# interactiveaudiolab/ppgs

Hardware: AMD Instinct MI355X
Metric: PPG frames/sec (whole node), mel repr, batch=32x1000 frames (higher is better)
Workload: dtype bf16; 1 GPU; configs[1]: mel representation, batch=32 x 1000 frames per GPU, audio resident in HBM -> (32,40,1000) fp32 posteriors in HBM; batch=32, frames=1000, per_gpu_batches=1, parallelism=utterance-sharded x1, no data-path collective

## Files before the change

### ppgs_amd/csrc/ppg_layer32.h

```cpp
#pragma once

#include "ppg_device.h"
#include "ppg_launch.h"

#include <type_traits>
#include <utility>

namespace {

constexpr float kLnEps32 = 1e-5f;
constexpr int HC = 128;

constexpr int tile_blocks(int hidt) { return hidt == 256 ? 5 : 3; }
template <int HIDT, int TBN_ = tile_blocks(HIDT)>
struct Geo {
    static_assert(HIDT == 256 || HIDT == 512, "hidden width");
    static constexpr int RB = HIDT / 128;
    static constexpr int KS = HIDT / 16;
    static constexpr int KH = KS / 16;
    static constexpr int TBN = TBN_;
    static constexpr int TOKS = 32 * TBN;
    static constexpr int HBUFS = TBN_ == tile_blocks(HIDT) ? 1 : 2;
    static constexpr int L_ACT = 0;
    static constexpr int L_H = TBN * KS * 1024;
    static constexpr int L_LNP1 = L_H + HBUFS * TBN * 8 * 1024;
    static constexpr int L_LNP2 = L_LNP1 + 3 * HIDT * 4;
    static constexpr int L_BQ = L_LNP2 + 3 * HIDT * 4;
    static constexpr int L_STATS = L_BQ + 3 * HIDT * 4;
    static constexpr int L_B1 = L_STATS + 2 * 4 * TOKS * 4;
};

__device__ __forceinline__ uint32_t lds_addr32(const void* p) {
    return (uint32_t)(uintptr_t)(const __attribute__((address_space(3))) void*)p;
}
template <int OFF>
__device__ __forceinline__ void ds_read128(u32x4& dst, uint32_t addr) {
    asm volatile("ds_read_b128 %0, %1 offset:%2" : "=v"(dst) : "v"(addr), "n"(OFF));
}
template <int N>
__device__ __forceinline__ void lgkm_wait32(u32x4& r) {
    asm volatile("s_waitcnt lgkmcnt(%1)" : "+v"(r) : "n"(N) : "memory");
    __builtin_amdgcn_sched_barrier(0);
}
template <int OFF>
__device__ __forceinline__ void gload128(u32x4& dst, uint32_t voff, const char* sbase) {
    asm volatile("global_load_dwordx4 %0, %1, %2 offset:%3" : "=v"(dst) : "v"(voff), "s"(sbase), "n"(OFF) : "memory");
}
template <int OFF>
__device__ __forceinline__ void gload128_acc(u32x4& dst, uint32_t voff, const char* sbase) {
    asm volatile("global_load_dwordx4 %0, %1, %2 offset:%3" : "=a"(dst) : "v"(voff), "s"(sbase), "n"(OFF) : "memory");
}
template <int K>
__device__ __forceinline__ void gload_frag(u32x4& dst, uint32_t voff, const char* base) {
    gload128<(K % 4) * 1024>(dst, voff, base + (K / 4) * 4096);
}
template <int K>
__device__ __forceinline__ void gload_frag_acc(u32x4& dst, uint32_t voff, const char* base) {
    gload128_acc<(K % 4) * 1024>(dst, voff, base + (K / 4) * 4096);
}
template <int COUNT>
__device__ __forceinline__ void vm_wait_all(u32x4 (&r)[COUNT]) {
    asm volatile("s_waitcnt vmcnt(0)" ::: "memory");
#pragma unroll
    for (int i = 0; i < COUNT; ++i) asm volatile("" : "+v"(r[i]));
    __builtin_amdgcn_sched_barrier(0);
}
__device__ __forceinline__ void glds16(const char* uniform_base, uint32_t lane_off, uint32_t lds_wave_addr) {
    const uint64_t b = reinterpret_cast<uint64_t>(uniform_base);
    const uint64_t base = ((uint64_t)(uint32_t)__builtin_amdgcn_readfirstlane((int)(b >> 32)) << 32) |
                          (uint64_t)(uint32_t)__builtin_amdgcn_readfirstlane((int)(uint32_t)b);
    asm volatile("s_mov_b32 m0, %2\n\ts_nop 0\n\tglobal_load_lds_dwordx4 %0, %1"
                 :: "v"(lane_off), "s"(base), "s"(__builtin_amdgcn_readfirstlane(lds_wave_addr)) : "memory", "m0");
}

template <class OFFS, int I, int N, int D, class USE>
__device__ __forceinline__ void stream_step(u32x4 (&ring)[D], uint32_t b0, uint32_t b1, USE& use) {
    if constexpr (I < N) {
        lgkm_wait32<(N - 1 - I < D - 1) ? (N - 1 - I) : (D - 1)>(ring[I % D]);
        use(std::integral_constant<int, I>{}, ring[I % D]);
        if constexpr (I + D < N) {
            constexpr int off = OFFS::at(I + D);
            if constexpr (off < 65536) ds_read128<off>(ring[I % D], b0); else ds_read128<off - 65536>(ring[I % D], b1);
        }
        stream_step<OFFS, I + 1, N, D>(ring, b0, b1, use);
    }
}
template <class OFFS, int I, int N, int D>
__device__ __forceinline__ void stream_prime(u32x4 (&ring)[D], uint32_t b0, uint32_t b1) {
    if constexpr (I < D && I < N) {
        constexpr int off = OFFS::at(I);
        if constexpr (off < 65536) ds_read128<off>(ring[I], b0); else ds_read128<off - 65536>(ring[I], b1);
        stream_prime<OFFS, I + 1, N, D>(ring, b0, b1);
    }
}
template <class OFFS, int N, int D, class USE>
__device__ __forceinline__ void stream(uint32_t b0, uint32_t b1, USE use) {
    u32x4 ring[D];
    stream_prime<OFFS, 0, N, D>(ring, b0, b1);
    stream_step<OFFS, 0, N, D>(ring, b0, b1, use);
}
template <int KS, int K0, int TB0, int NTB>
struct OffPanel { static constexpr int at(int i) { return ((TB0 + i % NTB) * KS + K0 + i / NTB) * 1024; } };
template <int TBN>
struct OffH { static constexpr int at(int i) { return ((i % TBN) * 8 + i / TBN) * 1024; } };

template <int TBN, int PAR>
struct OffH2 { static constexpr int at(int i) { return PAR * (TBN * 8 * 1024) + ((i % TBN) * 8 + i / TBN) * 1024; } };

struct OffChunk256 {
    static constexpr int at(int i) {
        constexpr int KS = Geo<256>::KS, HOFF = Geo<256>::L_H - Geo<256>::L_ACT;
        if (i < 48) return ((i % 3) * KS + i / 3) * 1024;
        if (i < 80) return ((3 + (i - 48) % 2) * KS + (i - 48) / 2) * 1024;
        if (i < 104) return HOFF + (((i - 80) % 3) * 8 + (i - 80) / 3) * 1024;
        return HOFF + ((3 + (i - 104) % 2) * 8 + (i - 104) / 2) * 1024;
    }
};

__device__ __forceinline__ void stat4(f32x2& sum2, f32x2& sq2, float v0, float v1, float v2, float v3) {
    const f32x2 a = {v0, v1}, b = {v2, v3};
    sum2 += a;
    sq2 = __builtin_elementwise_fma(a, a, sq2);
    sum2 += b;
    sq2 = __builtin_elementwise_fma(b, b, sq2);
}
__device__ __forceinline__ float hsum2(f32x2 v) {
    float r;
    asm("v_add_f32 %0, %1, %2" : "=v"(r) : "v"(v.x), "v"(v.y));
    return r;
}
__device__ __forceinline__ float pair_sum(float v) {
    auto b = __builtin_amdgcn_permlane32_swap(__float_as_uint(v), __float_as_uint(v), false, false);
    return __uint_as_float(b[0]) + __uint_as_float(b[1]);
}

template <class P, int HIDT, int TBS = tile_blocks(HIDT)>
__device__ __forceinline__ void panel_store(uint32_t pb0, int wave, int t, int rb, const f32x16& y) {
    using G = Geo<HIDT, TBS>;
#pragma unroll
    for (int s = 0; s < 2; ++s) {
        const u32x4 frag = u32x4{P::pack2(y[8 * s + 0], y[8 * s + 1]), P::pack2(y[8 * s + 2], y[8 * s + 3]),
                                 P::pack2(y[8 * s + 4], y[8 * s + 5]), P::pack2(y[8 * s + 6], y[8 * s + 7])};
        const uint32_t addr = pb0 + (uint32_t)((t * G::KS + 2 * G::RB * wave + 2 * rb + s) * 1024);
        asm volatile("ds_write_b128 %0, %1" :: "v"(addr), "v"(frag) : "memory");
    }
}

template <class P, int HIDT, int TBS = tile_blocks(HIDT)>
__device__ __forceinline__ void qkv_tail(const Layer32Args& a, char* smem, const int m0, u32x4 (&w1f)[16], u32x4 (&w2f)[16],
                                         const int nblk = TBS) {
    using G = Geo<HIDT, TBS>;
    constexpr int RB = G::RB, KS = G::KS, KH = G::KH, TB = G::TBN, TOKS = G::TOKS;
    constexpr int NSTEP = 3 * RB, NHS = NSTEP * KH;
    constexpr int NMMA = 16 * TB;
    constexpr int NU = 2 * TB;
    constexpr int USTRIDE = (NMMA - 16) / NU;
    const int lane = threadIdx.x & 63;
    const int wave = __builtin_amdgcn_readfirstlane(threadIdx.x >> 6);
    const int tok = lane & 31, hh = lane >> 5;
    const uint32_t voff = lane * 16;
    const uint32_t pb0 = lds_addr32(smem) + G::L_ACT + lane * 16, pb1 = pb0 + 65536;
    const int fbase = 32 * RB * wave;
    const f32x16 zero = {0.f, 0.f, 0.f, 0.f, 0.f, 0.f, 0.f, 0.f, 0.f, 0.f, 0.f, 0.f, 0.f, 0.f, 0.f, 0.f};
    asm volatile("s_waitcnt lgkmcnt(0)" ::: "memory");
    __syncthreads();
    const float* bq = reinterpret_cast<const float*>(smem + G::L_BQ);
    int vcol[TB][2];
    bool valigned[TB];
    bool regular = m0 + TOKS <= a.M && nblk == TB;
#pragma unroll
    for (int t = 0; t < TB; ++t) {
#pragma unroll
        for (int h = 0; h < 2; ++h) {
            const int mb = m0 + 32 * t + 16 * h;
            vcol[t][h] = -1;
            if (mb < a.M && t < nblk) {
                const int w = a.blk_win[mb >> 4];
                if (w >= 0) {
                    const int ttb = mb - a.win[w].tok_off;
                    vcol[t][h] = a.win[w].vt_off + (ttb >> 5) * 32 + 4 * ((ttb >> 4) & 1);
                }
            }
        }
        valigned[t] = vcol[t][0] >= 0 && vcol[t][1] == vcol[t][0] + 4 && (vcol[t][0] & 31) == 0;
        regular = regular && valigned[t];
    }
    const char* wq = a.wq_img + ((size_t)wave * 3 * RB * KS) * 1024;
    f32x16 acc[2][TB];
    auto bias_of = [&](auto step_tag, float4 (&b4)[4]) {
        constexpr int STEP = decltype(step_tag)::value, KIND = STEP / RB, RBI = STEP % RB;
        if constexpr (KIND < 2) {
#pragma unroll
            for (int q = 0; q < 4; ++q) b4[q] = *reinterpret_cast<const float4*>(bq + HIDT * KIND + 32 * RBI + fbase + 16 * hh + 4 * q);
        } else {
            const float bv = bq[2 * HIDT + pair_row(fbase + 32 * RBI + tok)];
            b4[0] = make_float4(bv, bv, bv, bv);
        }
    };
    auto bias_c = [&](auto step_tag) {
        constexpr int STEP = decltype(step_tag)::value;
        f32x16 cinit = zero;
        float4 bb[4];
        bias_of(step_tag, bb);
        if constexpr (STEP / RB < 2) {
#pragma unroll
            for (int q = 0; q < 4; ++q) { cinit[4 * q + 0] = bb[q].x; cinit[4 * q + 1] = bb[q].y; cinit[4 * q + 2] = bb[q].z; cinit[4 * q + 3] = bb[q].w; }
        } else {
#pragma unroll
            for (int k = 0; k < 16; ++k) cinit[k] = bb[0].x;
        }
        return cinit;
    };
    u32x4 held = u32x4{0u, 0u, 0u, 0u};
    auto unit = [&](auto step_tag, auto u_tag) {
        constexpr int STEP = decltype(step_tag)::value, U = decltype(u_tag)::value;
        constexpr int KIND = STEP / RB, RBI = STEP % RB, t = U / 2, s2 = U % 2;
        const f32x16& c = acc[STEP & 1][t];
        if (regular) {
            u32x4 r;
            if constexpr (KIND < 2) {
                r = u32x4{P::pack2(c[8 * s2 + 0], c[8 * s2 + 1]),
                          P::pack2(c[8 * s2 + 2], c[8 * s2 + 3]),
                          P::pack2(c[8 * s2 + 4], c[8 * s2 + 5]),
                          P::pack2(c[8 * s2 + 6], c[8 * s2 + 7])};
            } else {
                r = u32x4{P::pack2(c[4 * s2 + 0], c[4 * s2 + 1]), P::pack2(c[4 * s2 + 2], c[4 * s2 + 3]),
                          P::pack2(c[4 * (s2 + 2) + 0], c[4 * (s2 + 2) + 1]), P::pack2(c[4 * (s2 + 2) + 2], c[4 * (s2 + 2) + 3])};
            }
            if constexpr (s2 == 0) {
                held = r;
            } else {
                u32x4 lo, hi;
#pragma unroll
                for (int d = 0; d < 4; ++d) {
                    const auto sw = __builtin_amdgcn_permlane16_swap(held[d], r[d], false, false);
                    lo[d] = sw[0]; hi[d] = sw[1];
                }
                const int r16 = lane & 15, k16 = lane >> 4;
                if constexpr (KIND < 2) {
                    char* dst = a.qk_out + ((size_t)(m0 + 32 * t + r16) * 2 * HIDT + HIDT * KIND + 32 * RBI + fbase) * 2 + 16 * k16;
                    *reinterpret_cast<u32x4*>(dst) = lo;
                    *reinterpret_cast<u32x4*>(dst + (size_t)16 * 2 * HIDT * 2) = hi;
                } else {
                    char* dst = a.vt_out + ((size_t)(fbase + 32 * RBI + r16) * a.vt_ld + vcol[t][0]) * 2 + 16 * (2 * (k16 & 1) + (k16 >> 1));
                    *reinterpret_cast<u32x4*>(dst) = lo;
                    *reinterpret_cast<u32x4*>(dst + (size_t)16 * a.vt_ld * 2) = hi;
                }
            }
            return;
        }
        if constexpr (KIND < 2) {
            const int m = m0 + 32 * t + tok;
            if (m < a.M && t < nblk) {
                char* dst = a.qk_out + ((size_t)m * 2 * HIDT + HIDT * KIND + 32 * RBI + fbase + 16 * hh) * 2;
                *reinterpret_cast<u32x4*>(dst + 16 * s2) = u32x4{
                    P::pack2(c[8 * s2 + 0], c[8 * s2 + 1]), P::pack2(c[8 * s2 + 2], c[8 * s2 + 3]),
                    P::pack2(c[8 * s2 + 4], c[8 * s2 + 5]), P::pack2(c[8 * s2 + 6], c[8 * s2 + 7])};
            }
        } else {
            char* rowp = a.vt_out + (size_t)(fbase + 32 * RBI + tok) * a.vt_ld * 2;
            if (valigned[t]) {
                *reinterpret_cast<u32x4*>(rowp + (size_t)(vcol[t][0] + 16 * s2 + 8 * hh) * 2) = u32x4{
                    P::pack2(c[4 * s2 + 0], c[4 * s2 + 1]), P::pack2(c[4 * s2 + 2], c[4 * s2 + 3]),
                    P::pack2(c[4 * (s2 + 2) + 0], c[4 * (s2 + 2) + 1]), P::pack2(c[4 * (s2 + 2) + 2], c[4 * (s2 + 2) + 3])};
            } else if (vcol[t][s2] >= 0) {
#pragma unroll
                for (int e = 0; e < 2; ++e) {
                    const int q = 2 * s2 + e;
                    *reinterpret_cast<uint2*>(rowp + (size_t)(vcol[t][s2] + 8 * (2 * e + hh)) * 2) = make_uint2(
                        P::pack2(c[4 * q + 0], c[4 * q + 1]), P::pack2(c[4 * q + 2], c[4 * q + 3]));
                }
            }
        }
    };
    auto half_step = [&](auto hs_tag, u32x4 (&cur)[16], u32x4 (&nxt)[16]) {
        constexpr int HS = decltype(hs_tag)::value;
        constexpr int STEP = HS / KH, kh = HS % KH;
        constexpr bool SWAP = STEP / RB == 2;
        constexpr bool LAST = HS + 1 == NHS;
        constexpr bool EPI = kh == 0 && STEP > 0;
        const char* nbase = wq + (size_t)(LAST ? HS : HS + 1) * 16 * 1024;
        f32x16 cinit = zero;
        if constexpr (kh == 0) {
            cinit = bias_c(std::integral_constant<int, STEP>{});
#pragma unroll
            for (int k = 0; k < 16; ++k) asm volatile("" : "+v"(cinit[k]));
        }
        f32x16 (&c)[TB] = acc[STEP & 1];
        stream<OffPanel<KS, 16 * kh, 0, TB>, NMMA, 6>(pb0, pb1, [&](auto ic, const u32x4& bf) {
            constexpr int i = decltype(ic)::value;
            constexpr int ks = i / TB, tb = i % TB;
            if constexpr (ks == 0 && kh == 0) c[tb] = SWAP ? P::mma32(bf, cur[0], cinit) : P::mma32(cur[0], bf, cinit);
            else c[tb] = SWAP ? P::mma32(bf, cur[ks], c[tb]) : P::mma32(cur[ks], bf, c[tb]);
            if constexpr (!LAST && i < 16) gload_frag<i>(nxt[i], voff, nbase);
            if constexpr (EPI && i >= 16 && (i - 16) % USTRIDE == 0 && (i - 16) / USTRIDE < NU)
                unit(std::integral_constant<int, STEP - 1>{}, std::integral_constant<int, (i - 16) / USTRIDE>{});
        });
        if constexpr (!LAST) {
            if constexpr (EPI) {
                if (regular) asm volatile("s_waitcnt vmcnt(%0)" :: "n"(NU) : "memory");
                else asm volatile("s_waitcnt vmcnt(0)" ::: "memory");
            } else {
                asm volatile("s_waitcnt vmcnt(0)" ::: "memory");
            }
#pragma unroll
            for (int k = 0; k < 16; ++k) asm volatile("" : "+v"(nxt[k]));
            __builtin_amdgcn_sched_barrier(0);
        }
    };
    [&]<int... S>(std::integer_sequence<int, S...>) {
        ((S % 2 == 0 ? half_step(std::integral_constant<int, S>{}, w1f, w2f)
                     : half_step(std::integral_constant<int, S>{}, w2f, w1f)), ...);
    }(std::make_integer_sequence<int, NHS>{});
    (void)TOKS;
    [&]<int... U>(std::integer_sequence<int, U...>) {
        (unit(std::integral_constant<int, NSTEP - 1>{}, std::integral_constant<int, U>{}), ...);
    }(std::make_integer_sequence<int, NU>{});
}

}
```

### ppgs_amd/csrc/ppg_layer32.hip

```cpp
#include "ppg_layer32.h"

namespace {

template <class P, int HIDT, bool QKV, int TBS = tile_blocks(HIDT)>
__global__ __launch_bounds__(256) __attribute__((amdgpu_waves_per_eu(1, 1))) void layer32_kernel(Layer32Args a) {
    using G = Geo<HIDT, TBS>;
    constexpr int RB = G::RB, KS = G::KS, KH = G::KH, TB = G::TBN, TOKS = G::TOKS;
    constexpr int TBT = tile_blocks(HIDT);
    constexpr bool SUB = TBS != TBT;
    constexpr int NSUB = (TBT + TBS - 1) / TBS;
    static_assert(!SUB || (HIDT == 256 && TBS == 2), "sub-tile workgroups: hidden 256, two token blocks");
    extern __shared__ __attribute__((aligned(16))) char smem[];
    const int tid = threadIdx.x;
    const int lane = tid & 63;
    const int wave = __builtin_amdgcn_readfirstlane(tid >> 6);
    const int tok = lane & 31, hh = lane >> 5;
    const int tile = SUB ? (int)blockIdx.x / NSUB : (int)blockIdx.x;
    const int tb0 = SUB ? ((int)blockIdx.x % NSUB) * TBS : 0;
    const int nblk = SUB ? min(TBS, TBT - tb0) : TBS;
    auto gblock = [&](int t) { return SUB ? tb0 + (t < nblk ? t : -tb0) : t; };
    const int m0 = tile * (32 * TBT) + 32 * tb0;
    const int NCH = a.F / HC;
    const uint32_t lds0 = lds_addr32(smem);
    const uint32_t voff = lane * 16;
    const uint32_t pb0 = lds0 + G::L_ACT + lane * 16, pb1 = pb0 + 65536;
    const uint32_t hb0 = lds0 + G::L_H + lane * 16;
    float* lnp1 = reinterpret_cast<float*>(smem + G::L_LNP1);
    float* lnp2 = reinterpret_cast<float*>(smem + G::L_LNP2);
    float* stats = reinterpret_cast<float*>(smem + G::L_STATS);
    const int fbase = 32 * RB * wave;
    [[maybe_unused]] const char* wq_first = a.wq_img + ((size_t)wave * 3 * RB * KS) * 1024;

#ifdef PPG_FFN_TIMING
    auto pstamp = [&](int k) {
        if (a.dbg && blockIdx.x == 0 && lane == 0) a.dbg[128 + wave * 16 + k] = __builtin_amdgcn_s_memtime();
    };
#else
    auto pstamp = [&](int) {};
#endif
    pstamp(0);

    u32x4 w1f[16], w2f[16];
    auto load16 = [&](u32x4 (&wf)[16], const char* base) {
        [&]<int... K>(std::integer_sequence<int, K...>) { (gload_frag<K>(wf[K], voff, base), ...); }(std::make_integer_sequence<int, 16>{});
    };
    constexpr bool XPRE = HIDT == 256;
    constexpr int NRES = XPRE ? TB * RB * 2 : 1;
    u32x4 res[NRES];
    const bool xpre = XPRE && a.x_half;
    if (xpre) {
        const char* xbase = reinterpret_cast<const char*>(a.X) + ((size_t)tile * 4 + wave) * (TBT * RB * 2 * 1024);
        if constexpr (!SUB) {
            [&]<int... K>(std::integer_sequence<int, K...>) { (gload_frag<K>(res[K], voff, xbase), ...); }(std::make_integer_sequence<int, NRES>{});
        } else {
            [&]<int... K>(std::integer_sequence<int, K...>) {
                (gload_frag<K % (RB * 2)>(res[K], voff, xbase + (size_t)gblock(K / (RB * 2)) * (RB * 2 * 1024)), ...);
            }(std::make_integer_sequence<int, NRES>{});
        }
    }
    {
        const char* src = a.ao + (size_t)tile * (TBT * KS * 1024);
#pragma unroll
        for (int i = 0; i < TB * KS / 4; ++i) {
            const int p = 4 * i + wave;
            const int q = SUB ? gblock(p / KS) * KS + p % KS : p;
            glds16(src + (size_t)q * 1024, voff, lds0 + G::L_ACT + p * 1024);
        }
    }
    f32x16 yacc[RB][TB];
    {
        constexpr int NP = (3 * HIDT / 4 + 255) / 256;
        float4 p1[NP], p2[NP], pq[NP];
#pragma unroll
        for (int u = 0; u < NP; ++u) {
            const int i = min(tid + 256 * u, 3 * HIDT / 4 - 1);
            const int v = i / (HIDT / 4), j = i - v * (HIDT / 4);
            p1[u] = reinterpret_cast<const float4*>(v == 0 ? a.bo : (v == 1 ? a.g1 : a.e1))[j];
            p2[u] = reinterpret_cast<const float4*>(v == 0 ? a.b2 : (v == 1 ? a.g2 : a.e2))[j];
            if constexpr (QKV) pq[u] = reinterpret_cast<const float4*>(a.bq)[i];
        }
        constexpr int B1MAX = 8;
        float4 pb[B1MAX];
#pragma unroll
        for (int u = 0; u < B1MAX; ++u) pb[u] = reinterpret_cast<const float4*>(a.b1)[min(tid + 256 * u, a.F / 4 - 1)];
#pragma unroll
        for (int u = 0; u < NP; ++u) {
            const int i = tid + 256 * u;
            if (i < 3 * HIDT / 4) {
                reinterpret_cast<float4*>(lnp1)[i] = p1[u];
                reinterpret_cast<float4*>(lnp2)[i] = p2[u];
                if constexpr (QKV) reinterpret_cast<float4*>(smem + G::L_BQ)[i] = pq[u];
            }
        }
#pragma unroll
        for (int u = 0; u < B1MAX; ++u)
            if (tid + 256 * u < a.F / 4) reinterpret_cast<float4*>(smem + G::L_B1)[tid + 256 * u] = pb[u];
    }
    const f32x16 zero = {0.f, 0.f, 0.f, 0.f, 0.f, 0.f, 0.f, 0.f, 0.f, 0.f, 0.f, 0.f, 0.f, 0.f, 0.f, 0.f};
    [&]<int... R>(std::integer_sequence<int, R...>) {
        ([&] {
            constexpr int rbp = R / KH, kh = R % KH;
            const char* base = a.wo_img + ((size_t)wave * RB * KS) * 1024;
            load16(w1f, base + ((size_t)(2 * rbp) * KS + 16 * kh) * 1024);
            load16(w2f, base + ((size_t)(2 * rbp + 1) * KS + 16 * kh) * 1024);
            vm_wait_all(w1f);
            vm_wait_all(w2f);
            if constexpr (R == 0) {
#pragma unroll
                for (int k = 0; k < NRES; ++k) asm volatile("" : "+v"(res[k]));
                __syncthreads();
                pstamp(1);
            }
            if (!(PPG_DBG(a) & 1)) {
                stream<OffPanel<KS, 16 * kh, 0, TB>, 16 * TB, 6>(pb0, pb1, [&](auto ic, const u32x4& bf) {
                    constexpr int i = decltype(ic)::value;
                    constexpr int ks = i / TB, tb = i % TB;
                    if constexpr (ks == 0 && kh == 0) {
                        yacc[2 * rbp][tb] = P::mma32(w1f[0], bf, zero);
                        yacc[2 * rbp + 1][tb] = P::mma32(w2f[0], bf, zero);
                    } else {
                        yacc[2 * rbp][tb] = P::mma32(w1f[ks], bf, yacc[2 * rbp][tb]);
                        yacc[2 * rbp + 1][tb] = P::mma32(w2f[ks], bf, yacc[2 * rbp + 1][tb]);
                    }
                });
            }
        }(), ...);
    }(std::make_integer_sequence<int, (RB / 2) * KH>{});
    pstamp(2);

    float* xt = a.X + ((size_t)tile * 4 + wave) * (TBT * RB * 4 * 256) + lane * 4;
    char* xh = reinterpret_cast<char*>(a.X) + ((size_t)tile * 4 + wave) * (TBT * RB * 2 * 1024) + lane * 16;
    auto layer_norm = [&](auto residual_tag, auto xhalf_tag, const float* lnp, auto emit) {
        constexpr bool RES = decltype(residual_tag)::value;
        constexpr bool XH = decltype(xhalf_tag)::value;
        constexpr int STAMP = RES ? 7 : 9;
        constexpr bool KEEP = RB == 2;
        float4 bias4[KEEP ? RB : 1][4], gv[KEEP ? RB : 1][4], ev[KEEP ? RB : 1][4];
        auto quad = [&](int which, int rb, int q) { return *reinterpret_cast<const float4*>(lnp + which * HIDT + fbase + 32 * rb + 16 * hh + 4 * q); };
        if constexpr (KEEP) {
#pragma unroll
            for (int rb = 0; rb < RB; ++rb)
#pragma unroll
                for (int q = 0; q < 4; ++q) bias4[rb][q] = quad(0, rb, q);
        }
#pragma unroll
        for (int t = 0; t < TB; ++t) {
            f32x2 sum2 = {0.f, 0.f}, sq2 = {0.f, 0.f};
#pragma unroll
            for (int rb = 0; rb < RB; ++rb)
#pragma unroll
                for (int s2 = 0; s2 < 2; ++s2) {
                    float r8[8] = {0.f, 0.f, 0.f, 0.f, 0.f, 0.f, 0.f, 0.f};
                    [[maybe_unused]] uint32_t w4[4] = {0u, 0u, 0u, 0u};
                    if constexpr (RES && XH) {
                        u32x4 rv;
                        if constexpr (XPRE) rv = res[(t * RB + rb) * 2 + s2];
                        else rv = *reinterpret_cast<const u32x4*>(xh + ((gblock(t) * RB + rb) * 2 + s2) * 1024);
                        w4[0] = rv.x; w4[1] = rv.y; w4[2] = rv.z; w4[3] = rv.w;
                    } else if constexpr (RES) {
#pragma unroll
                        for (int e = 0; e < 2; ++e) {
                            const float4 rv = *reinterpret_cast<const float4*>(xt + ((gblock(t) * RB + rb) * 4 + 2 * s2 + e) * 256);
                            r8[4 * e + 0] = rv.x; r8[4 * e + 1] = rv.y; r8[4 * e + 2] = rv.z; r8[4 * e + 3] = rv.w;
                        }
                    }
#pragma unroll
                    for (int e = 0; e < 2; ++e) {
                        const int q = 2 * s2 + e;
                        float4 bv;
                        if constexpr (KEEP) bv = bias4[rb][q]; else bv = quad(0, rb, q);
                        if constexpr (RES && XH) {
                            const float bq4[4] = {bv.x, bv.y, bv.z, bv.w};
#pragma unroll
                            for (int k = 0; k < 4; ++k) {
                                const float sum = yacc[rb][t][4 * q + k] + bq4[k];
                                float out;
                                if (k & 1) asm("v_fma_mix_f32 %0, %1, 1.0, %2 op_sel:[1,0,0] op_sel_hi:[1,0,0]" : "=v"(out) : "v"(w4[2 * e + k / 2]), "v"(sum));
                                else asm("v_fma_mix_f32 %0, %1, 1.0, %2 op_sel:[0,0,0] op_sel_hi:[1,0,0]" : "=v"(out) : "v"(w4[2 * e + k / 2]), "v"(sum));
                                yacc[rb][t][4 * q + k] = out;
                            }
                        } else
                        {
                        yacc[rb][t][4 * q + 0] += bv.x + r8[4 * e + 0]; yacc[rb][t][4 * q + 1] += bv.y + r8[4 * e + 1];
                        yacc[rb][t][4 * q + 2] += bv.z + r8[4 * e + 2]; yacc[rb][t][4 * q + 3] += bv.w + r8[4 * e + 3];
                        }
                        stat4(sum2, sq2, yacc[rb][t][4 * q + 0], yacc[rb][t][4 * q + 1], yacc[rb][t][4 * q + 2], yacc[rb][t][4 * q + 3]);
                    }
                }
            const float sum = pair_sum(hsum2(sum2));
            const float sq = pair_sum(hsum2(sq2));
            if (hh == 0) {
                stats[wave * TOKS + 32 * t + tok] = sum;
                stats[4 * TOKS + wave * TOKS + 32 * t + tok] = sq;
            }
        }
        if constexpr (KEEP) {
#pragma unroll
            for (int rb = 0; rb < RB; ++rb)
#pragma unroll
                for (int q = 0; q < 4; ++q) { gv[rb][q] = quad(1, rb, q); ev[rb][q] = quad(2, rb, q); }
        }
        pstamp(STAMP);
        __syncthreads();
        pstamp(STAMP + 1);
#pragma unroll
        for (int t = 0; t < TB; ++t) {
            const float* s = stats + 32 * t + tok;
            const float mean = ((s[0] + s[TOKS]) + (s[2 * TOKS] + s[3 * TOKS])) * (1.0f / HIDT);
            const float ex2 = ((s[4 * TOKS] + s[5 * TOKS]) + (s[6 * TOKS] + s[7 * TOKS])) * (1.0f / HIDT);
            const float rstd = __builtin_amdgcn_rsqf(fmaxf(ex2 - mean * mean, 0.f) + kLnEps32);
            const float shift = -mean * rstd;
#pragma unroll
            for (int rb = 0; rb < RB; ++rb) {
#pragma unroll
                for (int q = 0; q < 4; ++q) {
                    float4 g4, e4;
                    if constexpr (KEEP) { g4 = gv[rb][q]; e4 = ev[rb][q]; } else { g4 = quad(1, rb, q); e4 = quad(2, rb, q); }
                    yacc[rb][t][4 * q + 0] = fmaf(fmaf(yacc[rb][t][4 * q + 0], rstd, shift), g4.x, e4.x);
                    yacc[rb][t][4 * q + 1] = fmaf(fmaf(yacc[rb][t][4 * q + 1], rstd, shift), g4.y, e4.y);
                    yacc[rb][t][4 * q + 2] = fmaf(fmaf(yacc[rb][t][4 * q + 2], rstd, shift), g4.z, e4.z);
                    yacc[rb][t][4 * q + 3] = fmaf(fmaf(yacc[rb][t][4 * q + 3], rstd, shift), g4.w, e4.w);
                }
                emit(t, rb, yacc[rb][t]);
            }
        }
    };
    auto panel_write = [&](int t, int rb, const f32x16& y) {
#pragma unroll
        for (int s = 0; s < 2; ++s) {
            const u32x4 frag = u32x4{P::pack2(y[8 * s + 0], y[8 * s + 1]), P::pack2(y[8 * s + 2], y[8 * s + 3]),
                                     P::pack2(y[8 * s + 4], y[8 * s + 5]), P::pack2(y[8 * s + 6], y[8 * s + 7])};
            const uint32_t addr = pb0 + (uint32_t)((t * KS + 2 * RB * wave + 2 * rb + s) * 1024);
            asm volatile("ds_write_b128 %0, %1" :: "v"(addr), "v"(frag) : "memory");
        }
    };
    if (a.x_half) layer_norm(std::true_type{}, std::true_type{}, lnp1, panel_write);
    else layer_norm(std::true_type{}, std::false_type{}, lnp1, panel_write);
    load16(w1f, a.w1_img + ((size_t)wave * KS) * 1024);
    asm volatile("s_waitcnt lgkmcnt(0)" ::: "memory");
    __syncthreads();
    pstamp(3);

    auto bias_read = [&](u32x4 (&braw)[4], int c) {
#pragma unroll
        for (int q = 0; q < 4; ++q) ds_read128<0>(braw[q], lds0 + G::L_B1 + (uint32_t)((c * HC + 32 * wave + 8 * q + 4 * hh) * 4));
    };
    auto bias_of = [&](u32x4 (&braw)[4]) {
        f32x16 bias;
#pragma unroll
        for (int q = 0; q < 4; ++q) {
            asm volatile("" : "+v"(braw[q]));
            bias[4 * q + 0] = __uint_as_float(braw[q].x); bias[4 * q + 1] = __uint_as_float(braw[q].y);
            bias[4 * q + 2] = __uint_as_float(braw[q].z); bias[4 * q + 3] = __uint_as_float(braw[q].w);
        }
        return bias;
    };
    if constexpr (SUB) {
        u32x4 w1g[16], w2g[16];
        f32x16 hacc[2][TB];
        u32x4 braw[4];
        auto h_write = [&](auto par_tag, auto t_tag, auto s_tag) {
            constexpr int par = decltype(par_tag)::value, t = decltype(t_tag)::value, s2 = decltype(s_tag)::value;
            const f32x16& hv = hacc[par][t];
            const u32x4 frag = u32x4{P::relu2(P::pack2(hv[8 * s2 + 0], hv[8 * s2 + 1])), P::relu2(P::pack2(hv[8 * s2 + 2], hv[8 * s2 + 3])),
                                     P::relu2(P::pack2(hv[8 * s2 + 4], hv[8 * s2 + 5])), P::relu2(P::pack2(hv[8 * s2 + 6], hv[8 * s2 + 7]))};
            const uint32_t addr = hb0 + (uint32_t)(par * (TB * 8 * 1024) + (t * 8 + 2 * wave + s2) * 1024);
            asm volatile("ds_write_b128 %0, %1" :: "v"(addr), "v"(frag) : "memory");
        };
        auto w1_of = [&](int c) { return a.w1_img + (((size_t)c * 4 + wave) * KS) * 1024; };
        auto w2_of = [&](int c) { return a.w2_img + (((size_t)c * 4 + wave) * RB * 8) * 1024; };
        const int nrun = (PPG_DBG(a) & 2) ? 0 : NCH;
        if (nrun > 0) {
            bias_read(braw, 0);
            asm volatile("s_waitcnt lgkmcnt(0)" ::: "memory");
            const f32x16 bias0 = bias_of(braw);
            vm_wait_all(w1f);
            const char* w1n = w1_of(nrun > 1 ? 1 : 0);
            const char* w20 = w2_of(0);
            stream<OffPanel<KS, 0, 0, TB>, 16 * TB, 6>(pb0, pb1, [&](auto ic, const u32x4& bf) {
                constexpr int i = decltype(ic)::value;
                constexpr int ks = i / TB, tb = i % TB;
                if constexpr (ks == 0) hacc[0][tb] = P::mma32(w1f[0], bf, bias0);
                else hacc[0][tb] = P::mma32(w1f[ks], bf, hacc[0][tb]);
                if constexpr (i < 16) gload_frag<i>(w1g[i], voff, w1n);
                else gload_frag_acc<i - 16>(w2f[i - 16], voff, w20);
                if constexpr (i == 20) bias_read(braw, nrun > 1 ? 1 : 0);
            });
        }
        auto iter = [&](auto par_tag, auto next_tag, int c) {
            constexpr int PAR = decltype(par_tag)::value;
            constexpr bool NEXT = decltype(next_tag)::value;
            u32x4 (&wa)[16] = *(PAR ? &w1f : &w1g);
            u32x4 (&wn)[16] = *(PAR ? &w1g : &w1f);
            u32x4 (&w2c)[16] = *(PAR ? &w2g : &w2f);
            u32x4 (&w2n)[16] = *(PAR ? &w2f : &w2g);
            const char* nx = c + 2 < NCH ? w1_of(c + 2) : (QKV ? wq_first : w1_of(c));
            const char* nx2 = w2_of(c + 1 < NCH ? c + 1 : c);
            const int cb = c + 2 < NCH ? c + 2 : c;
            f32x16 bias;
            if constexpr (NEXT) bias = bias_of(braw);
            asm volatile("s_waitcnt vmcnt(16)" ::: "memory");
#pragma unroll
            for (int k = 0; k < 16; ++k) asm volatile("" : "+v"(wa[k]));
            __builtin_amdgcn_sched_barrier(0);
            if constexpr (NEXT) {
                stream<OffPanel<KS, 0, 0, TB>, 16 * TB, 6>(pb0, pb1, [&](auto ic, const u32x4& bf) {
                    constexpr int i = decltype(ic)::value;
                    constexpr int ks = i / TB, tb = i % TB;
                    if constexpr (ks == 0) hacc[PAR ^ 1][tb] = P::mma32(wa[0], bf, bias);
                    else hacc[PAR ^ 1][tb] = P::mma32(wa[ks], bf, hacc[PAR ^ 1][tb]);
                    if constexpr (i % 2 == 0) gload_frag<i / 2>(wn[i / 2], voff, nx);
                    if constexpr (i % 4 == 1 && i / 4 < 2 * TB)
                        h_write(std::integral_constant<int, PAR>{}, std::integral_constant<int, (i / 4) / 2>{}, std::integral_constant<int, (i / 4) % 2>{});
                });
            } else {
                [&]<int... U>(std::integer_sequence<int, U...>) {
                    (h_write(std::integral_constant<int, PAR>{}, std::integral_constant<int, U / 2>{}, std::integral_constant<int, U % 2>{}), ...);
                }(std::make_integer_sequence<int, 2 * TB>{});
            }
            asm volatile("s_waitcnt lgkmcnt(0)" ::: "memory");
            asm volatile("s_barrier" ::: "memory");
            if constexpr (NEXT) asm volatile("s_waitcnt vmcnt(16)" ::: "memory");
            else asm volatile("s_waitcnt vmcnt(0)" ::: "memory");
#pragma unroll
            for (int k = 0; k < 16; ++k) asm volatile("" : "+a"(w2c[k]));
            __builtin_amdgcn_sched_barrier(0);
            stream<OffH2<TB, PAR>, 8 * TB, 6>(hb0, hb0, [&](auto ic, const u32x4& bf) {
                constexpr int i = decltype(ic)::value;
                constexpr int ks = i / TB, tb = i % TB;
                yacc[0][tb] = P::mma32(w2c[ks], bf, yacc[0][tb]);
                yacc[1][tb] = P::mma32(w2c[8 + ks], bf, yacc[1][tb]);
                if constexpr (NEXT) gload_frag_acc<i>(w2n[i], voff, nx2);
                if constexpr (i == 2) bias_read(braw, cb);
            });
        };
        for (int c = 0; c + 2 < nrun; c += 2) {
            iter(std::integral_constant<int, 0>{}, std::true_type{}, c);
            iter(std::integral_constant<int, 1>{}, std::true_type{}, c + 1);
        }
        if (nrun > 0) {
            iter(std::integral_constant<int, 0>{}, std::true_type{}, nrun - 2);
            iter(std::integral_constant<int, 1>{}, std::false_type{}, nrun - 1);
        }
    } else if constexpr (HIDT == 256) {
        u32x4 braw[4];
        u32x4 w2a[16];
        bias_read(braw, 0);
        asm volatile("s_waitcnt lgkmcnt(0)" ::: "memory");
        for (int c = 0; c < ((PPG_DBG(a) & 2) ? 0 : NCH); ++c) {
#ifdef PPG_FFN_TIMING
            auto cstamp = [&](int k) { if (c == 4 && a.dbg && blockIdx.x == 0 && lane == 0) a.dbg[wave * 8 + k] = __builtin_amdgcn_s_memtime(); };
#else
            auto cstamp = [&](int) {};
#endif
            cstamp(0);
            const f32x16 bias = bias_of(braw);
            vm_wait_all(w1f);
            const char* w2c = a.w2_img + (((size_t)c * 4 + wave) * RB * 8) * 1024;
            const char* next1 = c + 1 < NCH ? a.w1_img + (((size_t)(c + 1) * 4 + wave) * KS) * 1024
                                : (QKV ? wq_first : a.w1_img + (((size_t)c * 4 + wave) * KS) * 1024);
            const int cn = c + 1 < NCH ? c + 1 : c;
            f32x16 hacc[TB];
            auto h_write = [&](auto t_tag, auto s_tag) {
                constexpr int t = decltype(t_tag)::value, s2 = decltype(s_tag)::value;
                const u32x4 frag = u32x4{P::relu2(P::pack2(hacc[t][8 * s2 + 0], hacc[t][8 * s2 + 1])), P::relu2(P::pack2(hacc[t][8 * s2 + 2], hacc[t][8 * s2 + 3])),
                                         P::relu2(P::pack2(hacc[t][8 * s2 + 4], hacc[t][8 * s2 + 5])), P::relu2(P::pack2(hacc[t][8 * s2 + 6], hacc[t][8 * s2 + 7]))};
                const uint32_t addr = hb0 + (uint32_t)((t * 8 + 2 * wave + s2) * 1024);
                asm volatile("ds_write_b128 %0, %1" :: "v"(addr), "v"(frag) : "memory");
            };
            uint32_t hlo0 = 0, hlo1 = 0;
            auto h_half = [&](auto t_tag, auto s_tag, auto part_tag) {
                constexpr int t = decltype(t_tag)::value, s2 = decltype(s_tag)::value, part = decltype(part_tag)::value;
                if constexpr (part == 0) {
                    hlo0 = P::relu2(P::pack2(hacc[t][8 * s2 + 0], hacc[t][8 * s2 + 1]));
                    hlo1 = P::relu2(P::pack2(hacc[t][8 * s2 + 2], hacc[t][8 * s2 + 3]));
                } else {
                    const u32x4 frag = u32x4{hlo0, hlo1, P::relu2(P::pack2(hacc[t][8 * s2 + 4], hacc[t][8 * s2 + 5])), P::relu2(P::pack2(hacc[t][8 * s2 + 6], hacc[t][8 * s2 + 7]))};
                    const uint32_t addr = hb0 + (uint32_t)((t * 8 + 2 * wave + s2) * 1024);
                    asm volatile("ds_write_b128 %0, %1" :: "v"(addr), "v"(frag) : "memory");
                }
            };
            stream<OffChunk256, 120, 6>(pb0, pb1, [&](auto ic, const u32x4& bf) {
                constexpr int i = decltype(ic)::value;
                if constexpr (i < 48) {
                    constexpr int ks = i / 3, tb = i % 3;
                    if constexpr (ks == 0) P::mma32v0(hacc[tb], w1f[0], bf, bias);
                    else P::mma32v(hacc[tb], w1f[ks], bf);
                    if constexpr (i % 3 == 1) gload_frag_acc<i / 3>(w2a[i / 3], voff, w2c);
                } else if constexpr (i < 80) {
                    constexpr int j = i - 48, ks = j / 2, tb = 3 + j % 2;
                    if constexpr (j == 0) cstamp(1);
                    if constexpr (ks == 0) P::mma32v0(hacc[tb], w1f[0], bf, bias);
                    else P::mma32v(hacc[tb], w1f[ks], bf);
                    if constexpr (j == 4) asm volatile("" :: "v"(bias));
                    if constexpr (j >= 2 && (j - 2) % 3 < 2 && (j - 2) / 3 < 6)
                        h_half(std::integral_constant<int, ((j - 2) / 3) / 2>{}, std::integral_constant<int, ((j - 2) / 3) % 2>{}, std::integral_constant<int, (j - 2) % 3>{});
                    if constexpr (i == 74) asm volatile("s_barrier" ::: "memory");
                } else if constexpr (i < 104) {
                    constexpr int j = i - 80, ks = j / 3, tb = j % 3;
                    if constexpr (j == 0) {
                        cstamp(2);
                        asm volatile("s_waitcnt vmcnt(0)" ::: "memory");
#pragma unroll
                        for (int k = 0; k < 16; ++k) asm volatile("" : "+a"(w2a[k]));
                        __builtin_amdgcn_sched_barrier(0);
                    }
                    yacc[0][tb] = P::mma32(w2a[ks], bf, yacc[0][tb]);
                    yacc[1][tb] = P::mma32(w2a[8 + ks], bf, yacc[1][tb]);
                    if constexpr (j < 16) gload_frag<j>(w1f[j], voff, next1);
                    if constexpr (j % 3 == 1 && j / 3 < 4) h_write(std::integral_constant<int, 3 + (j / 3) / 2>{}, std::integral_constant<int, (j / 3) % 2>{});
                    if constexpr (j == 17) bias_read(braw, cn);
                    if constexpr (i == 98) asm volatile("s_barrier" ::: "memory");
                } else {
                    constexpr int j = i - 104, ks = j / 2, tb = 3 + j % 2;
                    if constexpr (j == 0) cstamp(3);
                    yacc[0][tb] = P::mma32(w2a[ks], bf, yacc[0][tb]);
                    yacc[1][tb] = P::mma32(w2a[8 + ks], bf, yacc[1][tb]);
                }
            });
            cstamp(5);
        }
    } else {
        for (int c = 0; c < ((PPG_DBG(a) & 2) ? 0 : NCH); ++c) {
#ifdef PPG_FFN_TIMING
            auto cstamp = [&](int k) { if (c == 4 && a.dbg && blockIdx.x == 0 && lane == 0) a.dbg[wave * 8 + k] = __builtin_amdgcn_s_memtime(); };
#else
            auto cstamp = [&](int) {};
#endif
            cstamp(0);
            f32x16 bias;
            {
                u32x4 braw[4];
#pragma unroll
                for (int q = 0; q < 4; ++q) ds_read128<0>(braw[q], lds0 + G::L_B1 + (uint32_t)((c * HC + 32 * wave + 8 * q + 4 * hh) * 4));
                asm volatile("s_waitcnt lgkmcnt(0)" ::: "memory");
#pragma unroll
                for (int q = 0; q < 4; ++q) {
                    asm volatile("" : "+v"(braw[q]));
                    bias[4 * q + 0] = __uint_as_float(braw[q].x); bias[4 * q + 1] = __uint_as_float(braw[q].y);
                    bias[4 * q + 2] = __uint_as_float(braw[q].z); bias[4 * q + 3] = __uint_as_float(braw[q].w);
                }
            }
            vm_wait_all(w1f);
            const char* w1c = a.w1_img + (((size_t)c * 4 + wave) * KS) * 1024;
            const char* w2c = a.w2_img + (((size_t)c * 4 + wave) * RB * 8) * 1024;
            const char* next1 = c + 1 < NCH ? a.w1_img + (((size_t)(c + 1) * 4 + wave) * KS) * 1024
                                : (QKV ? wq_first : w1c);
            f32x16 hacc[TB];
            auto h_write = [&](auto t_tag, auto s_tag) {
                constexpr int t = decltype(t_tag)::value, s2 = decltype(s_tag)::value;
                const u32x4 frag = u32x4{P::relu2(P::pack2(hacc[t][8 * s2 + 0], hacc[t][8 * s2 + 1])), P::relu2(P::pack2(hacc[t][8 * s2 + 2], hacc[t][8 * s2 + 3])),
                                         P::relu2(P::pack2(hacc[t][8 * s2 + 4], hacc[t][8 * s2 + 5])), P::relu2(P::pack2(hacc[t][8 * s2 + 6], hacc[t][8 * s2 + 7]))};
                const uint32_t addr = hb0 + (uint32_t)((t * 8 + 2 * wave + s2) * 1024);
                asm volatile("ds_write_b128 %0, %1" :: "v"(addr), "v"(frag) : "memory");
            };
                stream<OffPanel<KS, 0, 0, TB>, 16 * TB, 6>(pb0, pb1, [&](auto ic, const u32x4& bf) {
                    constexpr int i = decltype(ic)::value;
                    constexpr int ks = i / TB, tb = i % TB;
                    if constexpr (ks == 0) hacc[tb] = P::mma32(w1f[0], bf, bias);
                    else hacc[tb] = P::mma32(w1f[ks], bf, hacc[tb]);
                    if constexpr (i % 3 == 1) gload_frag<16 + i / 3>(w2f[i / 3], voff, w1c);
                });
                vm_wait_all(w2f);
                cstamp(1);
                stream<OffPanel<KS, 16, 0, TB>, 16 * TB, 6>(pb0, pb1, [&](auto ic, const u32x4& bf) {
                    constexpr int i = decltype(ic)::value;
                    constexpr int ks = i / TB, tb = i % TB;
                    if constexpr (i == 0) __builtin_amdgcn_s_barrier();
                    hacc[tb] = P::mma32(w2f[ks], bf, hacc[tb]);
                    if constexpr (i % 3 == 1) gload_frag<i / 3>(w1f[i / 3], voff, w2c);
                });
                cstamp(2);
                [&]<int... U>(std::integer_sequence<int, U...>) {
                    (h_write(std::integral_constant<int, U / 2>{}, std::integral_constant<int, U % 2>{}), ...);
                }(std::make_integer_sequence<int, 2 * TB>{});
                asm volatile("s_waitcnt lgkmcnt(0)" ::: "memory");
                cstamp(3);
                __syncthreads();
                cstamp(4);
                vm_wait_all(w1f);
                stream<OffH<TB>, 8 * TB, 6>(hb0, hb0, [&](auto ic, const u32x4& bf) {
                    constexpr int i = decltype(ic)::value;
                    constexpr int ks = i / TB, tb = i % TB;
                    yacc[0][tb] = P::mma32(w1f[ks], bf, yacc[0][tb]);
                    yacc[1][tb] = P::mma32(w1f[8 + ks], bf, yacc[1][tb]);
                    if constexpr (i < 16) gload_frag<16 + i>(w2f[i], voff, w2c);
                });
                vm_wait_all(w2f);
                stream<OffH<TB>, 8 * TB, 6>(hb0, hb0, [&](auto ic, const u32x4& bf) {
                    constexpr int i = decltype(ic)::value;
                    constexpr int ks = i / TB, tb = i % TB;
                    yacc[2][tb] = P::mma32(w2f[ks], bf, yacc[2][tb]);
                    yacc[3][tb] = P::mma32(w2f[8 + ks], bf, yacc[3][tb]);
                    if constexpr (i < 16) gload_frag<i>(w1f[i], voff, next1);
                });
            cstamp(5);
        }
    }
    vm_wait_all(w1f);
    pstamp(4);

    layer_norm(std::false_type{}, std::false_type{}, lnp2, [&](int t, int rb, const f32x16& y) {
        if (SUB && t >= nblk) {
        } else if (a.write_x && a.x_half) {
#pragma unroll
            for (int s2 = 0; s2 < 2; ++s2)
                *reinterpret_cast<u32x4*>(xh + ((gblock(t) * RB + rb) * 2 + s2) * 1024) = u32x4{pack_f16x2(y[8 * s2 + 0], y[8 * s2 + 1]), pack_f16x2(y[8 * s2 + 2], y[8 * s2 + 3]),
                                                                                  pack_f16x2(y[8 * s2 + 4], y[8 * s2 + 5]), pack_f16x2(y[8 * s2 + 6], y[8 * s2 + 7])};
        } else if (a.write_x) {
#pragma unroll
            for (int q = 0; q < 4; ++q)
                *reinterpret_cast<float4*>(xt + ((gblock(t) * RB + rb) * 4 + q) * 256) = make_float4(y[4 * q + 0], y[4 * q + 1], y[4 * q + 2], y[4 * q + 3]);
        }
        if constexpr (QKV) panel_write(t, rb, y);
        const int m = m0 + 32 * t + tok;
        if (a.Xb && m < a.M && !(SUB && t >= nblk)) {
            char* brow = a.Xb + ((size_t)m * HIDT + fbase + 32 * rb + 16 * hh) * 2;
#pragma unroll
            for (int s = 0; s < 2; ++s)
                *reinterpret_cast<u32x4*>(brow + 16 * s) = u32x4{P::pack2(y[8 * s + 0], y[8 * s + 1]), P::pack2(y[8 * s + 2], y[8 * s + 3]),
                                                                  P::pack2(y[8 * s + 4], y[8 * s + 5]), P::pack2(y[8 * s + 6], y[8 * s + 7])};
        }
    });
    pstamp(5);

    if constexpr (QKV) {
        qkv_tail<P, HIDT, TBS>(a, smem, m0, w1f, w2f, nblk);
        pstamp(6);
    }
}

template <class P, int HIDT>
hipError_t launch_layer32_h(const Layer32Args& a, hipStream_t s) {
    if (a.F % HC || a.F < HC || a.M <= 0 || a.F > 8192) return hipErrorInvalidValue;
    auto launch = [&](auto kern, auto geo, int subs) {
        using G = decltype(geo);
        const size_t lds = (size_t)G::L_B1 + (size_t)a.F * 4;
        if (lds > 163840) return hipErrorInvalidValue;
        const int tiles = (a.M + 32 * tile_blocks(HIDT) - 1) / (32 * tile_blocks(HIDT));
        static ppg::LdsLimit limit;
        const hipError_t e = limit.ensure(reinterpret_cast<const void*>(kern), lds);
        if (e != hipSuccess) return e;
        hipLaunchKernelGGL(kern, dim3(tiles * subs), dim3(256), lds, s, a);
        return hipGetLastError();
    };
    if constexpr (HIDT == 256) {
        if (a.sub_tiles) {
            if ((a.F / HC) % 2) return hipErrorInvalidValue;
            if (a.wq_img != nullptr) return launch(layer32_kernel<P, HIDT, true, 2>, Geo<HIDT, 2>{}, 3);
            return launch(layer32_kernel<P, HIDT, false, 2>, Geo<HIDT, 2>{}, 3);
        }
    }
    if (a.wq_img != nullptr) return launch(layer32_kernel<P, HIDT, true>, Geo<HIDT>{}, 1);
    return launch(layer32_kernel<P, HIDT, false>, Geo<HIDT>{}, 1);
}

template <class P>
hipError_t launch_layer32_p(const Layer32Args& a, hipStream_t s) {
    if (a.H == 256) return launch_layer32_h<P, 256>(a, s);
    if (a.H == 512) return launch_layer32_h<P, 512>(a, s);
    return hipErrorInvalidValue;
}

}

namespace ppg {

int layer32_tokens(int hidden) { return hidden == 512 ? Geo<512>::TOKS : Geo<256>::TOKS; }

hipError_t launch_layer32(int precision, const Layer32Args& a, hipStream_t s) {
    if (precision == PPG_PRECISION_BF16) return launch_layer32_p<PrecBF16>(a, s);
    if (precision == PPG_PRECISION_FP16) return launch_layer32_p<PrecF16>(a, s);
    return hipErrorInvalidValue;
}

}
```

Measured before the change: 48.01 million frames/s.

## Pipeline layer32 prologue per token block for hidden-256 tiles

For hidden width 256 without sub-tiles, the kernel prologue becomes a per-token-block software pipeline. Activation panels and residual fragments for upcoming blocks are prefetched with double buffering while the current block runs its output projection, residual add and layernorm, and parameter and bias loads are pushed into later stages. A separate change in qkv_tail reads the window tables through constant address space and moves the barrier after the index computation so that work overlaps the LDS wait. The goal is to hide global-load latency in the prologue, at the cost of more registers, hand-counted vmcnt waits that must stay correct, and a much more complex code path.

```diff
diff --git a/ppgs_amd/csrc/ppg_layer32.h b/ppgs_amd/csrc/ppg_layer32.h
--- a/ppgs_amd/csrc/ppg_layer32.h
+++ b/ppgs_amd/csrc/ppg_layer32.h
@@ -162,9 +162,8 @@
     const uint32_t pb0 = lds_addr32(smem) + G::L_ACT + lane * 16, pb1 = pb0 + 65536;
     const int fbase = 32 * RB * wave;
     const f32x16 zero = {0.f, 0.f, 0.f, 0.f, 0.f, 0.f, 0.f, 0.f, 0.f, 0.f, 0.f, 0.f, 0.f, 0.f, 0.f, 0.f};
-    asm volatile("s_waitcnt lgkmcnt(0)" ::: "memory");
-    __syncthreads();
-    const float* bq = reinterpret_cast<const float*>(smem + G::L_BQ);
+    const auto* blk_win = (const __attribute__((address_space(4))) int*)a.blk_win;
+    const auto* win = (const __attribute__((address_space(4))) std::remove_pointer_t<decltype(a.win)>*)a.win;
     int vcol[TB][2];
     bool valigned[TB];
     bool regular = m0 + TOKS <= a.M && nblk == TB;
@@ -175,16 +174,19 @@
             const int mb = m0 + 32 * t + 16 * h;
             vcol[t][h] = -1;
             if (mb < a.M && t < nblk) {
-                const int w = a.blk_win[mb >> 4];
+                const int w = blk_win[mb >> 4];
                 if (w >= 0) {
-                    const int ttb = mb - a.win[w].tok_off;
-                    vcol[t][h] = a.win[w].vt_off + (ttb >> 5) * 32 + 4 * ((ttb >> 4) & 1);
+                    const int ttb = mb - win[w].tok_off;
+                    vcol[t][h] = win[w].vt_off + (ttb >> 5) * 32 + 4 * ((ttb >> 4) & 1);
                 }
             }
         }
         valigned[t] = vcol[t][0] >= 0 && vcol[t][1] == vcol[t][0] + 4 && (vcol[t][0] & 31) == 0;
         regular = regular && valigned[t];
     }
+    asm volatile("s_waitcnt lgkmcnt(0)" ::: "memory");
+    __syncthreads();
+    const float* bq = reinterpret_cast<const float*>(smem + G::L_BQ);
     const char* wq = a.wq_img + ((size_t)wave * 3 * RB * KS) * 1024;
     f32x16 acc[2][TB];
     auto bias_of = [&](auto step_tag, float4 (&b4)[4]) {
diff --git a/ppgs_amd/csrc/ppg_layer32.hip b/ppgs_amd/csrc/ppg_layer32.hip
--- a/ppgs_amd/csrc/ppg_layer32.hip
+++ b/ppgs_amd/csrc/ppg_layer32.hip
@@ -45,20 +45,22 @@
         [&]<int... K>(std::integer_sequence<int, K...>) { (gload_frag<K>(wf[K], voff, base), ...); }(std::make_integer_sequence<int, 16>{});
     };
     constexpr bool XPRE = HIDT == 256;
-    constexpr int NRES = XPRE ? TB * RB * 2 : 1;
+    constexpr bool PIPE = HIDT == 256 && !SUB;
+    constexpr int RPB = RB * 2;
+    constexpr int NRES = PIPE ? 2 * RPB : (XPRE ? TB * RPB : 1);
     u32x4 res[NRES];
     const bool xpre = XPRE && a.x_half;
-    if (xpre) {
-        const char* xbase = reinterpret_cast<const char*>(a.X) + ((size_t)tile * 4 + wave) * (TBT * RB * 2 * 1024);
-        if constexpr (!SUB) {
-            [&]<int... K>(std::integer_sequence<int, K...>) { (gload_frag<K>(res[K], voff, xbase), ...); }(std::make_integer_sequence<int, NRES>{});
-        } else {
-            [&]<int... K>(std::integer_sequence<int, K...>) {
-                (gload_frag<K % (RB * 2)>(res[K], voff, xbase + (size_t)gblock(K / (RB * 2)) * (RB * 2 * 1024)), ...);
-            }(std::make_integer_sequence<int, NRES>{});
-        }
-    }
-    {
+    if constexpr (!PIPE) {
+        if (xpre) {
+            const char* xbase = reinterpret_cast<const char*>(a.X) + ((size_t)tile * 4 + wave) * (TBT * RB * 2 * 1024);
+            if constexpr (!SUB) {
+                [&]<int... K>(std::integer_sequence<int, K...>) { (gload_frag<K>(res[K], voff, xbase), ...); }(std::make_integer_sequence<int, NRES>{});
+            } else {
+                [&]<int... K>(std::integer_sequence<int, K...>) {
+                    (gload_frag<K % (RB * 2)>(res[K], voff, xbase + (size_t)gblock(K / (RB * 2)) * (RB * 2 * 1024)), ...);
+                }(std::make_integer_sequence<int, NRES>{});
+            }
+        }
         const char* src = a.ao + (size_t)tile * (TBT * KS * 1024);
 #pragma unroll
         for (int i = 0; i < TB * KS / 4; ++i) {
@@ -68,7 +70,7 @@
         }
     }
     f32x16 yacc[RB][TB];
-    {
+    if constexpr (!PIPE) {
         constexpr int NP = (3 * HIDT / 4 + 255) / 256;
         float4 p1[NP], p2[NP], pq[NP];
 #pragma unroll
@@ -97,7 +99,7 @@
             if (tid + 256 * u < a.F / 4) reinterpret_cast<float4*>(smem + G::L_B1)[tid + 256 * u] = pb[u];
     }
     const f32x16 zero = {0.f, 0.f, 0.f, 0.f, 0.f, 0.f, 0.f, 0.f, 0.f, 0.f, 0.f, 0.f, 0.f, 0.f, 0.f, 0.f};
-    [&]<int... R>(std::integer_sequence<int, R...>) {
+    if constexpr (!PIPE) [&]<int... R>(std::integer_sequence<int, R...>) {
         ([&] {
             constexpr int rbp = R / KH, kh = R % KH;
             const char* base = a.wo_img + ((size_t)wave * RB * KS) * 1024;
@@ -126,7 +128,7 @@
             }
         }(), ...);
     }(std::make_integer_sequence<int, (RB / 2) * KH>{});
-    pstamp(2);
+    if constexpr (!PIPE) pstamp(2);
 
     float* xt = a.X + ((size_t)tile * 4 + wave) * (TBT * RB * 4 * 256) + lane * 4;
     char* xh = reinterpret_cast<char*>(a.X) + ((size_t)tile * 4 + wave) * (TBT * RB * 2 * 1024) + lane * 16;
@@ -234,9 +236,179 @@
             asm volatile("ds_write_b128 %0, %1" :: "v"(addr), "v"(frag) : "memory");
         }
     };
-    if (a.x_half) layer_norm(std::true_type{}, std::true_type{}, lnp1, panel_write);
-    else layer_norm(std::true_type{}, std::false_type{}, lnp1, panel_write);
-    load16(w1f, a.w1_img + ((size_t)wave * KS) * 1024);
+    if constexpr (PIPE) {
+        static_assert(RB == 2 && KH == 1 && KS % 4 == 0 && 3 * HIDT / 4 <= 256, "pipelined prologue: hidden 256");
+        constexpr int PPB = KS / 4;
+        const char* xbase = reinterpret_cast<const char*>(a.X) + ((size_t)tile * 4 + wave) * (TBT * RPB * 1024);
+        const char* aosrc = a.ao + (size_t)tile * (TBT * KS * 1024);
+        auto req_res = [&](auto t_tag) {
+            constexpr int t = decltype(t_tag)::value;
+            if (xpre)
+                [&]<int... K>(std::integer_sequence<int, K...>) {
+                    (gload_frag<K>(res[(t % 2) * RPB + K], voff, xbase + t * (RPB * 1024)), ...);
+                }(std::make_integer_sequence<int, RPB>{});
+        };
+        auto req_panel = [&](auto t_tag, auto i_tag) {
+            constexpr int t = decltype(t_tag)::value, i = decltype(i_tag)::value;
+            const int p = t * KS + 4 * i + wave;
+            glds16(aosrc + (size_t)p * 1024, voff, lds0 + G::L_ACT + p * 1024);
+        };
+        auto req_panel_all = [&](auto t_tag) {
+            [&]<int... I>(std::integer_sequence<int, I...>) { (req_panel(t_tag, std::integral_constant<int, I>{}), ...); }(std::make_integer_sequence<int, PPB>{});
+        };
+        auto quad1 = [&](int which, int rb, int q) { return *reinterpret_cast<const float4*>(lnp1 + which * HIDT + fbase + 32 * rb + 16 * hh + 4 * q); };
+        req_res(std::integral_constant<int, 0>{});
+        req_panel_all(std::integral_constant<int, 0>{});
+        {
+            const char* base = a.wo_img + ((size_t)wave * RB * KS) * 1024;
+            load16(w1f, base);
+            load16(w2f, base + (size_t)KS * 1024);
+        }
+        u32x4 p1r;
+        {
+            const int i = min(tid, 3 * HIDT / 4 - 1);
+            const int v = i / (HIDT / 4), j = i - v * (HIDT / 4);
+            const float4* psrc = reinterpret_cast<const float4*>(v == 0 ? a.bo : (v == 1 ? a.g1 : a.e1)) + j;
+            asm volatile("global_load_dwordx4 %0, %1, off" : "=v"(p1r) : "v"(psrc) : "memory");
+        }
+        req_res(std::integral_constant<int, 1>{});
+        req_panel_all(std::integral_constant<int, 1>{});
+        auto pass1 = [&](auto t_tag, auto xhalf_tag) {
+            constexpr int t = decltype(t_tag)::value;
+            constexpr bool XH = decltype(xhalf_tag)::value;
+            f32x2 sum2 = {0.f, 0.f}, sq2 = {0.f, 0.f};
+#pragma unroll
+            for (int rb = 0; rb < RB; ++rb)
+#pragma unroll
+                for (int s2 = 0; s2 < 2; ++s2) {
+                    float r8[8] = {0.f, 0.f, 0.f, 0.f, 0.f, 0.f, 0.f, 0.f};
+                    [[maybe_unused]] uint32_t w4[4] = {0u, 0u, 0u, 0u};
+                    if constexpr (XH) {
+                        const u32x4 rv = res[(t % 2) * RPB + rb * 2 + s2];
+                        w4[0] = rv.x; w4[1] = rv.y; w4[2] = rv.z; w4[3] = rv.w;
+                    } else {
+#pragma unroll
+                        for (int e = 0; e < 2; ++e) {
+                            const float4 rv = *reinterpret_cast<const float4*>(xt + ((t * RB + rb) * 4 + 2 * s2 + e) * 256);
+                            r8[4 * e + 0] = rv.x; r8[4 * e + 1] = rv.y; r8[4 * e + 2] = rv.z; r8[4 * e + 3] = rv.w;
+                        }
+                    }
+#pragma unroll
+                    for (int e = 0; e < 2; ++e) {
+                        const int q = 2 * s2 + e;
+                        const float4 bv = quad1(0, rb, q);
+                        if constexpr (XH) {
+                            const float bq4[4] = {bv.x, bv.y, bv.z, bv.w};
+#pragma unroll
+                            for (int k = 0; k < 4; ++k) {
+                                const float sum = yacc[rb][t][4 * q + k] + bq4[k];
+                                float out;
+                                if (k & 1) asm("v_fma_mix_f32 %0, %1, 1.0, %2 op_sel:[1,0,0] op_sel_hi:[1,0,0]" : "=v"(out) : "v"(w4[2 * e + k / 2]), "v"(sum));
+                                else asm("v_fma_mix_f32 %0, %1, 1.0, %2 op_sel:[0,0,0] op_sel_hi:[1,0,0]" : "=v"(out) : "v"(w4[2 * e + k / 2]), "v"(sum));
+                                yacc[rb][t][4 * q + k] = out;
+                            }
+                        } else {
+                            yacc[rb][t][4 * q + 0] += bv.x + r8[4 * e + 0]; yacc[rb][t][4 * q + 1] += bv.y + r8[4 * e + 1];
+                            yacc[rb][t][4 * q + 2] += bv.z + r8[4 * e + 2]; yacc[rb][t][4 * q + 3] += bv.w + r8[4 * e + 3];
+                        }
+                        stat4(sum2, sq2, yacc[rb][t][4 * q + 0], yacc[rb][t][4 * q + 1], yacc[rb][t][4 * q + 2], yacc[rb][t][4 * q + 3]);
+                    }
+                }
+            const float sum = pair_sum(hsum2(sum2));
+            const float sq = pair_sum(hsum2(sq2));
+            if (hh == 0) {
+                stats[wave * TOKS + 32 * t + tok] = sum;
+                stats[4 * TOKS + wave * TOKS + 32 * t + tok] = sq;
+            }
+        };
+        auto pass2 = [&](auto t_tag) {
+            constexpr int t = decltype(t_tag)::value;
+            const float* s = stats + 32 * t + tok;
+            const float mean = ((s[0] + s[TOKS]) + (s[2 * TOKS] + s[3 * TOKS])) * (1.0f / HIDT);
+            const float ex2 = ((s[4 * TOKS] + s[5 * TOKS]) + (s[6 * TOKS] + s[7 * TOKS])) * (1.0f / HIDT);
+            const float rstd = __builtin_amdgcn_rsqf(fmaxf(ex2 - mean * mean, 0.f) + kLnEps32);
+            const float shift = -mean * rstd;
+#pragma unroll
+            for (int rb = 0; rb < RB; ++rb) {
+#pragma unroll
+                for (int q = 0; q < 4; ++q) {
+                    const float4 g4 = quad1(1, rb, q), e4 = quad1(2, rb, q);
+                    yacc[rb][t][4 * q + 0] = fmaf(fmaf(yacc[rb][t][4 * q + 0], rstd, shift), g4.x, e4.x);
+                    yacc[rb][t][4 * q + 1] = fmaf(fmaf(yacc[rb][t][4 * q + 1], rstd, shift), g4.y, e4.y);
+                    yacc[rb][t][4 * q + 2] = fmaf(fmaf(yacc[rb][t][4 * q + 2], rstd, shift), g4.z, e4.z);
+                    yacc[rb][t][4 * q + 3] = fmaf(fmaf(yacc[rb][t][4 * q + 3], rstd, shift), g4.w, e4.w);
+                }
+                panel_write(t, rb, yacc[rb][t]);
+            }
+        };
+        [&]<int... T>(std::integer_sequence<int, T...>) {
+            ([&] {
+                constexpr int t = T;
+                const std::integral_constant<int, t> t_tag{};
+                if constexpr (t + 1 < TB) {
+                    if (xpre) asm volatile("s_waitcnt vmcnt(%0)" :: "n"(RPB + PPB) : "memory");
+                    else asm volatile("s_waitcnt vmcnt(%0)" :: "n"(PPB) : "memory");
+                } else {
+                    asm volatile("s_waitcnt vmcnt(0)" ::: "memory");
+                }
+                if constexpr (t == 0) {
+#pragma unroll
+                    for (int k = 0; k < 16; ++k) asm volatile("" : "+v"(w1f[k]));
+#pragma unroll
+                    for (int k = 0; k < 16; ++k) asm volatile("" : "+v"(w2f[k]));
+                    asm volatile("" : "+v"(p1r));
+                }
+#pragma unroll
+                for (int k = 0; k < RPB; ++k) asm volatile("" : "+v"(res[(t % 2) * RPB + k]));
+                __builtin_amdgcn_sched_barrier(0);
+                pstamp(10 + t);
+                if constexpr (t == 0) {
+                    if (tid < 3 * HIDT / 4) reinterpret_cast<u32x4*>(lnp1)[tid] = p1r;
+                    asm volatile("s_waitcnt lgkmcnt(0)" ::: "memory");
+                }
+                asm volatile("s_barrier" ::: "memory");
+                if constexpr (t == 0) pstamp(1);
+                stream<OffPanel<KS, 0, t, 1>, KS, 6>(pb0, pb1, [&](auto ic, const u32x4& bf) {
+                    constexpr int ks = decltype(ic)::value;
+                    if (!(PPG_DBG(a) & 1)) {
+                        if constexpr (ks == 0) {
+                            yacc[0][t] = P::mma32(w1f[0], bf, zero);
+                            yacc[1][t] = P::mma32(w2f[0], bf, zero);
+                        } else {
+                            yacc[0][t] = P::mma32(w1f[ks], bf, yacc[0][t]);
+                            yacc[1][t] = P::mma32(w2f[ks], bf, yacc[1][t]);
+                        }
+                    }
+                    if constexpr (t + 2 < TB && ks % 2 == 1 && ks / 2 < PPB)
+                        req_panel(std::integral_constant<int, t + 2>{}, std::integral_constant<int, ks / 2>{});
+                });
+                if constexpr (t + 1 == TB) {
+                    pstamp(2);
+                    if (wave < 3) {
+                        glds16(reinterpret_cast<const char*>(wave == 0 ? a.b2 : (wave == 1 ? a.g2 : a.e2)), voff, lds0 + G::L_LNP2 + wave * 1024);
+                        if constexpr (QKV) glds16(reinterpret_cast<const char*>(a.bq) + wave * 1024, voff, lds0 + G::L_BQ + wave * 1024);
+                    }
+                    const int b1k = a.F / 256;
+#pragma unroll
+                    for (int u = 0; u < 8; ++u)
+                        if (4 * u + wave < b1k) glds16(reinterpret_cast<const char*>(a.b1) + (4 * u + wave) * 1024, voff, lds0 + G::L_B1 + (4 * u + wave) * 1024);
+                    if ((a.F & 255) && tid < 32) reinterpret_cast<float4*>(smem + G::L_B1)[b1k * 64 + tid] = reinterpret_cast<const float4*>(a.b1)[b1k * 64 + tid];
+                    load16(w1f, a.w1_img + ((size_t)wave * KS) * 1024);
+                }
+                if (a.x_half) pass1(t_tag, std::true_type{});
+                else pass1(t_tag, std::false_type{});
+                if constexpr (t + 2 < TB) req_res(std::integral_constant<int, t + 2>{});
+                asm volatile("s_waitcnt lgkmcnt(0)" ::: "memory");
+                asm volatile("s_barrier" ::: "memory");
+                pass2(t_tag);
+            }(), ...);
+        }(std::make_integer_sequence<int, TB>{});
+        asm volatile("s_waitcnt vmcnt(16)" ::: "memory");
+    } else {
+        if (a.x_half) layer_norm(std::true_type{}, std::true_type{}, lnp1, panel_write);
+        else layer_norm(std::true_type{}, std::false_type{}, lnp1, panel_write);
+        load16(w1f, a.w1_img + ((size_t)wave * KS) * 1024);
+    }
     asm volatile("s_waitcnt lgkmcnt(0)" ::: "memory");
     __syncthreads();
     pstamp(3);
```

Result: no change. 48.17 million frames/s (median of 6 runs) (+0.3%).
